# DassHydro-dev/smash

Measured on AMD Instinct MI355X. Metric: cell-timesteps/s, forward+adjoint sweep, higher is better.
Workload: dtype f32

## Files before the change

smash_amd/csrc/smashx.hip:

```cpp
#include "../../include/smashx.h"

#include <hip/hip_runtime.h>
#include <rccl/rccl.h>

#include <dlfcn.h>

#include <algorithm>
#include <functional>
#include <numeric>
#include <cstdio>
#include <cstdlib>
#include <cstring>
#include <string>
#include <vector>

#include "sx_cost.h"
#include "sx_jreg.h"
#include "sx_kernels.h"
#include "sx_ensemble.h"
#include "sx_resident.h"
#include "sx_fields.h"
#include "sx_interception.h"
#include "sx_meanforcing.h"
#include "sx_prcpindices.h"
// ... 199 lines not shown
}

__global__ void k_gauge_rows(float* dst, const float* src, const int* gid, int ng, int nt) {
    const int t = blockIdx.x * blockDim.x + threadIdx.x, g = blockIdx.y;
    if (t < nt && g < ng) dst[(size_t)g * nt + t] = src[(size_t)gid[g] * nt + t];
}


struct RcclApi {
    void* h = nullptr;
    std::string err;
    decltype(&ncclGetUniqueId) GetUniqueId = nullptr;
    decltype(&ncclCommInitRank) CommInitRank = nullptr;
    decltype(&ncclCommDestroy) CommDestroy = nullptr;
    decltype(&ncclSend) Send = nullptr;
    decltype(&ncclRecv) Recv = nullptr;
    decltype(&ncclAllReduce) AllReduce = nullptr;
    decltype(&ncclGroupStart) GroupStart = nullptr;
    decltype(&ncclGroupEnd) GroupEnd = nullptr;
    decltype(&ncclGetErrorString) GetErrorString = nullptr;
    decltype(&ncclCommCount) CommCount = nullptr;
    decltype(&ncclGetVersion) GetVersion = nullptr;
    bool ok() const { return h != nullptr && err.empty(); }
};
RcclApi& rccl() {
    static RcclApi R;
    static bool tried = false;
    if (tried) return R;
    tried = true;
    const char* names[] = {getenv("SMASHX_RCCL_LIB"), "librccl.so.1", "librccl.so", "/opt/rocm/lib/librccl.so.1"};
    for (const char* n : names) {
        if (!n || !n[0]) continue;
        R.h = dlopen(n, RTLD_NOW | RTLD_LOCAL);
        if (R.h) break;
    }
    if (!R.h) { R.err = std::string("librccl.so.1 not found: ") + (dlerror() ? dlerror() : ""); return R; }
#define SX_SYM(f) do { R.f = (decltype(R.f))dlsym(R.h, "nccl" #f); if (!R.f) R.err = "librccl lacks nccl" #f; } while (0)
    SX_SYM(GetUniqueId); SX_SYM(CommInitRank); SX_SYM(CommDestroy); SX_SYM(Send); SX_SYM(Recv); SX_SYM(AllReduce);
    SX_SYM(GroupStart); SX_SYM(GroupEnd); SX_SYM(GetErrorString);
#undef SX_SYM
    R.CommCount = (decltype(R.CommCount))dlsym(R.h, "ncclCommCount");
    R.GetVersion = (decltype(R.GetVersion))dlsym(R.h, "ncclGetVersion");
    return R;
}
#define NCCLCHK(expr)                                                                                   \
    do {                                                                                                \
        ncclResult_t r_ = (expr);                                                                       \
        if (r_ != ncclSuccess)                                                                          \
            return fail(SMASHX_E_HIP, std::string(#expr) + ": " + rccl().GetErrorString(r_) + " (" + __FILE__ + ":" + std::to_string(__LINE__) + ")"); \
    } while (0)

struct SxComm {
    ncclComm_t comm = nullptr;
    int rank = 0, nranks = 1, device = -1;
    hipStream_t stream = nullptr;
    double* d_buf = nullptr;
    std::vector<smashx_plan*> plans;
};
struct PeerSeg { int rank, first, count; };

struct Launch { hipEvent_t a, b; int kind; double cellsteps; };

}

struct smashx_plan {
    smashx_config cfg{};
    SxSchedule sch;
    int n = 0, npad = 0, nt = 0, ng = 0, st = 0;
    long n2 = 0;
    int M = 0;
    int Tc = 0, nchunks = 0;
    bool have_forcing = false, have_options = false, have_qobs = false, uploaded = false;
    bool chunk_ready = false, adj_ready = false;
    smashx_options opt{};
    std::vector<float> wgauge;
    hipStream_t stream = nullptr;
    hipStream_t stream_r = nullptr;
    int Tp = 0;
    bool hi_tape = true;
    int chain_from = 1;
    bool chain_stage = false; SxStageTables stg{}; int stg_blocks = 0, stg_rows_extra = 0; size_t stg_lds = 0;
    float* hrk = nullptr; bool hrk_tried = false, early_adj = true;
    size_t vlds_fwd = 0, vlds_adj = 0;
    std::vector<hipEvent_t> buf_free;
    std::vector<double> round_ncells;
    bool chain_used = false;
    bool chain = true;
    int n_out = 0, n_in = 0;
    int *d_out_x = nullptr, *d_in_x = nullptr;
    float *halo_out = nullptr, *halo_in = nullptr;
    smashx_halo_fn halo_fn = nullptr; void* halo_user = nullptr;
    SxComm* xcomm = nullptr;
    std::vector<PeerSeg> out_segs, in_segs;
    int *d_out_xp = nullptr, *d_in_xp = nullptr;
    float *x_out = nullptr, *x_in = nullptr;
    float* x_keep = nullptr; size_t x_keep_cap = 0;
    std::vector<void*> allocs; std::vector<size_t> alloc_bytes;
    double bytes = 0;
    double hbm_free_at_plan = -1.0, hbm_total = -1.0;
    SxDeviceArrays A{};
    int* d_cell_flat = nullptr;
    int* d_sparse_idx = nullptr;
    float last_jobs_d = 0.f, last_jreg_d = 0.f;
    long n_sparse = 0;
    float* d_stage = nullptr;
    long stage_planes = 0;
    float* d_full[SX_NFIELDS] = {nullptr};
    float* st0[SX_NSSLOTS] = {nullptr};
    float* ckpt = nullptr;
    float* d_prcp = nullptr; float* d_pet = nullptr;
    int* d_ctrl_pos = nullptr; double* d_ctrl = nullptr; size_t ctrl_cap = 0;
    smashx_forcing_layout flay{};
    unsigned short* d_prcp16 = nullptr; float* d_petd = nullptr; float* d_ratio = nullptr; unsigned* d_fstatus = nullptr;
    int ndays = 0; bool petd_open = false;
    std::vector<char> block_seen;
    int ngc = 0;
    std::vector<int> gauge_gid;
    int *d_gauge_gid = nullptr, *d_gauge_flwacc = nullptr;
    float *d_area = nullptr, *d_wgauge = nullptr, *d_qobs = nullptr, *d_qsim_b = nullptr, *d_cost_out = nullptr;
    SxGaugeSums* d_sums = nullptr; SxCostCoef* d_coef = nullptr;
    float* d_med = nullptr; int* d_med_idx = nullptr;
    int med_nslots = 0; int* d_med_slot = nullptr; float* d_medx = nullptr; int* d_medx_idx = nullptr;
    smashx_reduce_fn med_fn = nullptr; void* med_user = nullptr; std::vector<int> med_slot_h;
    float jobs = 0.f;
    struct Signature {
        bool have = false, have_mask = false, ready = false;
        std::vector<float> h_po; std::vector<int> h_mask;
        int maxev_cap = -1;
        int obs_s0 = -1, obs_lds = -1;
        SxSigArgs a{};
        float* d_po = nullptr; int *d_nev = nullptr, *d_ev = nullptr;
        float *d_probe_b = nullptr, *d_probe_gb = nullptr, *d_probe_gd = nullptr, *d_probe_keep = nullptr;
    } sig;
    std::vector<float> h_qobs;
    float* h_qsim_domain = nullptr; float* h_net_prcp_domain = nullptr; int dom_sparse = 0;
    bool dom_q_active = false;
    bool tan_ready = false;
    float* d_qsim_d = nullptr;
    float* d_tanplane[SMASHX_GNP + SMASHX_GNS] = {nullptr};
    bool tiled = false;
    int* d_active = nullptr;
    hipStream_t stream_j = nullptr;
    hipEvent_t ev_j = nullptr;
    float* d_jx[SMASHX_GNP + SMASHX_GNS] = {nullptr};
    float* d_jb[SMASHX_GNP + SMASHX_GNS] = {nullptr};
    float* d_jg[SMASHX_GNP + SMASHX_GNS] = {nullptr};
    float* d_jterm = nullptr; size_t jterm_planes = 0;
    float* d_jsum = nullptr;
    SxJregChains jchains{};
    bool jr_ready = false;
    std::vector<Launch> launches;
    std::vector<hipEvent_t> pool; size_t pool_used = 0;
    hipEvent_t ev0 = nullptr, ev1 = nullptr;
    smashx_timing timing{};
    int last_adjoint = 0;
    std::vector<signed char> h_flwdir;
    std::vector<signed char> h_flwdir_grid;
    struct MeanForcing {
        int state = 0;
        std::string refusal;
        std::vector<int> count;
        std::vector<int> begin;
        std::vector<int> h_list;
        int *d_list = nullptr, *d_begin = nullptr;
        float *d_state = nullptr, *d_mp = nullptr, *d_me = nullptr;
    } mf;
// ... 178 lines not shown
        if ((rc = p->dmalloc(&p->A.xT, (size_t)std::max(p->sch.nxslots, 1) * Tc))) return rc;
        HIPCHK(hipMemsetAsync(p->A.qtT, 0, (size_t)p->npad * Tc * 4, p->stream));
        HIPCHK(hipMemsetAsync(p->A.xT, 0, (size_t)std::max(p->sch.nxslots, 1) * Tc * 4, p->stream));
        p->chunk_ready = true;
    }
    if (p->h_qsim_domain && !p->A.qdT) {
        int rc;
        if ((rc = p->dmalloc(&p->A.qdT, (size_t)p->npad * p->Tc))) return rc;
    }
    if (adjoint && !p->adj_ready) {
        int rc;
        const size_t cs = (size_t)p->npad * p->Tc;
        if (p->A.qsk) { p->dfree(p->A.qsk); p->A.qsk = nullptr; }
        {
            const char* e = getenv("SMASHX_HR_SKEW");
            p->A.hr_skew = e ? atoi(e) != 0 : true;
            if ((rc = p->dmalloc(&p->A.hrT, cs))) return rc;
        }
        if ((rc = p->dmalloc(&p->A.tape_hp, cs))) return rc;
        if ((rc = p->dmalloc(&p->A.tape_hft, cs))) return rc;
        if (st == 5 || ((st == 2 || st == 3) && p->hi_tape)) { if ((rc = p->dmalloc(&p->A.tape_hi, cs))) return rc; }
        else if (st == 2 || st == 3) { if ((rc = p->dmalloc(&p->A.ckpt_hi, cs / SX_HIK))) return rc; }
        if (st == 3) { if ((rc = p->dmalloc(&p->A.tape_hst, cs))) return rc; }
        if (p->nchunks > 1) { if ((rc = p->dmalloc(&p->ckpt, (size_t)p->nchunks * SX_NSSLOTS * p->npad))) return rc; }
        for (int s = 0; s < SX_NSLOTS; ++s) if ((rc = p->dmalloc(&slot_vecs(p, s).grad, (size_t)p->npad))) return rc;
        if ((rc = p->dmalloc(&p->A.qgb, (size_t)std::max(p->ngc, 1) * p->nt))) return rc;
        if ((rc = p->dmalloc(&p->d_qsim_b, (size_t)std::max(p->ng, 1) * p->nt))) return rc;
        p->adj_ready = true;
    }
    if (p->A.ncs > 0 && !p->A.qsk) {
        const size_t need = (size_t)p->A.ncs * 16 * ((size_t)p->Tc / 4 + p->stg_rows_extra + 1);
        size_t fr = 0, tot = 0;
        HIPCHK(hipMemGetInfo(&fr, &tot));
        if ((double)fr > (double)need + 2.0e9) { int rc; if ((rc = p->dmalloc(&p->A.qsk, need / 4))) return rc; }
    }
    if (adjoint && !p->hrk_tried) {
        p->hrk_tried = true;
        const int cf = chain_first(p);
        const char* e = getenv("SMASHX_KEEP_CHAIN_TAPE");
        const bool want = e ? atoi(e) != 0 : true;
        if (const char* ea = getenv("SMASHX_EARLY_ADJ_CHAIN")) p->early_adj = atoi(ea) != 0;
        if (want && p->nchunks > 1 && cf < p->sch.nrounds && !p->tiled && p->n_in == 0 && p->n_out == 0 && p->Tp >= p->Tc) {
            const int kcs0 = p->sch.g_slot_begin[p->sch.round_group_begin[cf]], kncs = p->sch.nslots - kcs0;
            const size_t need = (size_t)(p->nchunks - 1) * (size_t)(p->Tc / 4) * (size_t)kncs * 16;
            size_t fr = 0, tot = 0;
            HIPCHK(hipMemGetInfo(&fr, &tot));
            if (kncs > 0 && (double)fr > (double)need + 2.0e9) {
                int rc; if ((rc = p->dmalloc(&p->hrk, need / 4))) return rc;
                p->A.kcs0 = kcs0; p->A.kncs = kncs;
            }
        }
    }
    return 0;
}

SxDeviceArrays view_at(const smashx_plan* p, int off) {
    SxDeviceArrays B = p->A;
    B.k0 = 0; B.k1 = p->n;
    const size_t q = (size_t)(off / 4);
    B.qtT = p->A.qtT + q * p->npad * 4;
    B.hrk = nullptr;
    if (p->A.hrT) { if (p->A.hr_skew) B.hr_row0 = (int)q; else B.hrT = p->A.hrT + q * p->npad * 4; }
    if (p->A.qdT) B.qdT = p->A.qdT + q * p->npad * 4;
    if (!p->chain) B.qsk = nullptr;
    B.xT = p->A.xT + q * p->A.nx * 4;
    if (p->A.qtdT) B.qtdT = p->A.qtdT + q * p->npad * 4;
    if (p->A.xdT) B.xdT = p->A.xdT + q * p->A.nx * 4;
    if (p->A.tape_hp) B.tape_hp = p->A.tape_hp + (size_t)off * p->npad;
    if (p->A.tape_hft) B.tape_hft = p->A.tape_hft + (size_t)off * p->npad;
    if (p->A.tape_hi) B.tape_hi = p->A.tape_hi + (size_t)off * p->npad;
    if (p->A.ckpt_hi) B.ckpt_hi = p->A.ckpt_hi + (size_t)(off / SX_HIK) * p->npad;
    if (p->A.tape_hst) B.tape_hst = p->A.tape_hst + (size_t)off * p->npad;
    return B;
}

typedef void (*VertKernel)(SxDeviceArrays, int, int);
VertKernel vert_fwd_kernel(int st, bool tape, bool compact) {
#define SX_GR(ST) {sx_k_vert_fwd<ST, false, false>, sx_k_vert_fwd<ST, false, true>, sx_k_vert_fwd<ST, true, false>, sx_k_vert_fwd<ST, true, true>}
    static const VertKernel k[5][4] = {SX_GR(1), SX_GR(2), SX_GR(3), SX_GR(4),
                                       {sx_k_vert_fwd_vic<false, false>, sx_k_vert_fwd_vic<false, true>, sx_k_vert_fwd_vic<true, false>, sx_k_vert_fwd_vic<true, true>}};
#undef SX_GR
    return k[st - 1][2 * tape + compact];
}
VertKernel vert_adj_kernel(int st, bool compact) {
    static const VertKernel k[5][2] = {{sx_k_vert_adj<1, false>, sx_k_vert_adj<1, true>}, {sx_k_vert_adj<2, false>, sx_k_vert_adj<2, true>},
                                       {sx_k_vert_adj<3, false>, sx_k_vert_adj<3, true>}, {sx_k_vert_adj<4, false>, sx_k_vert_adj<4, true>},
                                       {sx_k_vert_adj_vic<false>, sx_k_vert_adj_vic<true>}};
    return k[st - 1][compact];
}
VertKernel vert_tan_kernel(int st) {
    static const VertKernel k[5] = {sx_k_vert_fwd_d<1>, sx_k_vert_fwd_d<2>, sx_k_vert_fwd_d<3>, sx_k_vert_fwd_d<4>, sx_k_vert_fwd_vic_d};
    return k[st - 1];
}
void launch_vert(smashx_plan* p, VertKernel k, int kind, size_t lds, int off, int t0, int T) {
    const SxDeviceArrays B = view_at(p, off);
    if (B.k1 <= B.k0) return;
    const dim3 grid((B.k1 - B.k0 + SX_VBLOCK - 1) / SX_VBLOCK), block(SX_VBLOCK);
    p->mark_begin(kind, p->stream, (double)(B.k1 - B.k0) * T);
    hipLaunchKernelGGL(k, grid, block, lds, p->stream, B, t0, T);
    p->mark_end();
}
void vert_fwd(smashx_plan* p, int off, bool tape, int t0, int T) {
    launch_vert(p, vert_fwd_kernel(p->st, tape, p->A.prcp16 != nullptr), 0, p->st == 5 ? 0 : p->vlds_fwd, off, t0, T);
}
void vert_adj(smashx_plan* p, int off, int t0, int T) {
    launch_vert(p, vert_adj_kernel(p->st, p->A.prcp16 != nullptr), 3, p->st == 5 ? 0 : p->vlds_adj, off, t0, T);
}
void vert_tan(smashx_plan* p, int off, int t0, int T) { launch_vert(p, vert_tan_kernel(p->st), 0, 0, off, t0, T); }
double round_cells(const smashx_plan* p, int r0, int r1) {
    double c = 0.0;
    for (int r = r0; r < r1; ++r) c += p->round_ncells[r];
    return c;
}
int chain_first(const smashx_plan* p) {
    const int nr = p->sch.nrounds;
    return (p->chain && nr - p->chain_from >= 2) ? p->chain_from : nr;
}
void reset_chain_counters(smashx_plan* p, hipStream_t st) {
    (void)hipMemsetAsync(p->A.prog, 0, (size_t)p->sch.ngroups * sizeof(int), st);
    (void)hipMemsetAsync(p->A.prog + p->sch.ngroups + 1, 0, sizeof(int), st);
}
void route_fwd_rounds(smashx_plan* p, int off, bool tape, int t0, int T, hipStream_t st, int r0, int r1, int tan = 0) {
    SxDeviceArrays B = view_at(p, off);
    if (!p->dom_q_active) B.qdT = nullptr;
    if (tan) B.qsk = nullptr;
    const size_t lds = (size_t)2 * p->M * sizeof(float4);
    void (*const k)(SxDeviceArrays, int, int, int, int) = tan == 1 ? sx_k_route_fwd<true, false, 1> : tan == 2 ? sx_k_route_fwd<false, false, 2>
                                                         : tape ? sx_k_route_fwd<true, false> : sx_k_route_fwd<false, false>;
    for (int r = r0; r < r1; ++r) {
        const int g0 = p->sch.round_group_begin[r], ngr = p->sch.round_group_begin[r + 1] - g0;
        p->mark_begin(1, st, round_cells(p, r, r + 1) * T);
        hipLaunchKernelGGL(k, dim3(ngr), dim3(p->M), lds, st, B, g0, g0 + ngr, t0, T);
        p->mark_end();
    }
}
bool route_fwd_chained(smashx_plan* p, int off, bool tape, int t0, int T, hipStream_t st, hipEvent_t inputs_read = nullptr, float* hrk = nullptr) {
    const int nr = p->sch.nrounds, cf = chain_first(p);
    if (cf >= nr) return false;
    SxDeviceArrays B = view_at(p, off);
    if (hrk) { B.hrk = hrk; B.hr_row0 = 0; tape = true; }
    if (!p->dom_q_active) B.qdT = nullptr;
    const size_t lds = (size_t)2 * p->M * sizeof(float4);
    const int g0 = p->sch.round_group_begin[cf], g1 = p->sch.ngroups;
    reset_chain_counters(p, st);
    const int grid = g1 - g0;
    p->mark_begin(5, st, round_cells(p, cf, nr) * T);
    if (B.qsk)
        hipLaunchKernelGGL((sx_k_chain_transpose<true>), dim3((p->stg_blocks + SX_STG_WAVES - 1) / SX_STG_WAVES), dim3(64 * SX_STG_WAVES), p->stg_lds * SX_STG_WAVES, st, B, p->stg, g0, (T + SX_BT - 1) / SX_BT, p->stg_blocks, (int)p->stg_lds);
    const bool early = B.qsk && inputs_read && !B.qdT;
    if (early) (void)hipEventRecord(inputs_read, st);
    if (tape) hipLaunchKernelGGL((sx_k_route_fwd<true, true>), dim3(grid), dim3(p->M), lds, st, B, g0, g1, t0, T);
    else      hipLaunchKernelGGL((sx_k_route_fwd<false, true>), dim3(grid), dim3(p->M), lds, st, B, g0, g1, t0, T);
    p->mark_end();
    p->chain_used = true;
    return early;
}
void route_adj_chained(smashx_plan* p, int off, int t0, int T, hipStream_t st, float* hrk = nullptr, bool launch = true, bool copy = true) {
    const int nr = p->sch.nrounds, cf = chain_first(p);
    if (cf >= nr) return;
    SxDeviceArrays B = view_at(p, off);
    if (hrk) { B.hrk = hrk; B.hr_row0 = 0; }
    const size_t lds = (size_t)2 * p->M * sizeof(float4);
    const int g0 = p->sch.round_group_begin[cf], g1 = p->sch.ngroups;
    const int grid = g1 - g0;
    if (launch) {
        reset_chain_counters(p, st);
        p->mark_begin(6, st, round_cells(p, cf, nr) * T);
        hipLaunchKernelGGL((sx_k_route_adj<true>), dim3(grid), dim3(p->M), lds, st, B, g0, g1, t0, T);
        p->mark_end();
        p->chain_used = true;
    }
    if (copy && B.qsk) {
        p->mark_begin(7, st);
        hipLaunchKernelGGL((sx_k_chain_transpose<false>), dim3((p->stg_blocks + SX_STG_WAVES - 1) / SX_STG_WAVES), dim3(64 * SX_STG_WAVES), p->stg_lds * SX_STG_WAVES, st, B, p->stg, g0, (T + SX_BT - 1) / SX_BT, p->stg_blocks, (int)p->stg_lds);
        p->mark_end();
    }
}
void route_adj_rounds(smashx_plan* p, int off, int t0, int T, hipStream_t st) {
    const SxDeviceArrays B = view_at(p, off);
    const size_t lds = (size_t)2 * p->M * sizeof(float4);
    const int cf = chain_first(p);
    for (int r = cf - 1; r >= 0; --r) {
        const int g0 = p->sch.round_group_begin[r], ngr = p->sch.round_group_begin[r + 1] - g0;
        p->mark_begin(2, st, round_cells(p, r, r + 1) * T);
        hipLaunchKernelGGL((sx_k_route_adj<false>), dim3(ngr), dim3(p->M), lds, st, B, g0, g0 + ngr, t0, T);
        p->mark_end();
    }
}

// ... 80 lines not shown
        sizes[0] = (int)sizeof(smashx_config); sizes[1] = (int)sizeof(smashx_mesh); sizes[2] = (int)sizeof(smashx_options);
        sizes[3] = (int)sizeof(smashx_parameters); sizes[4] = (int)sizeof(smashx_states); sizes[5] = (int)sizeof(smashx_costs);
        sizes[6] = (int)sizeof(smashx_timing);
    }
    return SMASHX_ABI_VERSION;
}

int smashx_device_count(void) {
    int n = 0;
    if (hipGetDeviceCount(&n) != hipSuccess) return 0;
    return n;
}

int smashx_plan_create(const smashx_config* cfg, const smashx_mesh* mesh, smashx_plan** out) {
    if (!cfg || !mesh || !out) return fail(SMASHX_E_ARG, "null argument");
    *out = nullptr;
    if (cfg->structure < 1 || cfg->structure > 5) return fail(SMASHX_E_UNSUPPORTED, "structure must be gr-a/b/c/d or vic-a");
    if (cfg->nrow <= 0 || cfg->ncol <= 0 || cfg->nt <= 0 || cfg->ng < 0 || !(cfg->dt > 0.f) || !(cfg->dx > 0.f))
        return fail(SMASHX_E_ARG, "bad sizes in smashx_config");
    if (!mesh->flwdir || !mesh->flwacc || !mesh->active_cell || (cfg->ng > 0 && (!mesh->gauge_pos || !mesh->area)))
        return fail(SMASHX_E_ARG, "null mesh array");
    int ndev = 0;
    if (hipGetDeviceCount(&ndev) != hipSuccess || ndev <= 0)
        return fail(SMASHX_E_NODEVICE, "no HIP device: libsmashx has no CPU fallback");
    smashx_plan* p = new smashx_plan();
    p->cfg = *cfg;
    if (set_device(p)) { delete p; return SMASHX_E_HIP; }
    p->M = cfg->group_size > 0 ? cfg->group_size : 512;
    if (p->M % 64 != 0 || p->M > SX_MAXGROUP || p->M < 64) { delete p; return fail(SMASHX_E_ARG, "group_size must be a multiple of 64 in [64, 512]"); }
    const bool rect_tile = cfg->tile[1] > cfg->tile[0] && cfg->tile[3] > cfg->tile[2];
    const bool tiled = rect_tile || mesh->owner_mask;
    const int rc0 = sx_build_schedule(cfg->nrow, cfg->ncol, mesh->flwdir, mesh->active_cell, cfg->ng, mesh->gauge_pos, p->M,
                                      rect_tile ? cfg->tile : nullptr, p->sch, mesh->owner_mask, sublevels_env());
    if (rc0 != 0) { std::string e = p->sch.error; delete p; return fail(rc0 == -5 ? SMASHX_E_MESH : SMASHX_E_ARG, e); }
    p->tiled = tiled;
    if (!tiled) {
        p->h_flwdir.resize((size_t)cfg->nrow * cfg->ncol);
        for (size_t c = 0; c < p->h_flwdir.size(); ++c) { const int d = mesh->flwdir[c]; p->h_flwdir[c] = (d >= 1 && d <= 8 && mesh->active_cell[c] == 1) ? (signed char)d : 0; }
        p->h_flwdir_grid.resize(p->h_flwdir.size());
        for (size_t c = 0; c < p->h_flwdir_grid.size(); ++c) { const int d = mesh->flwdir[c]; p->h_flwdir_grid[c] = (d >= 1 && d <= 8) ? (signed char)d : 0; }
    }
    p->n = p->sch.n; p->npad = (p->n + SX_VBLOCK - 1) / SX_VBLOCK * SX_VBLOCK;
    p->nt = cfg->nt; p->ng = cfg->ng; p->st = cfg->structure; p->n2 = (long)cfg->nrow * cfg->ncol;
    int rc = 0;
#define TRY(x) do { rc = (x); if (rc) { smashx_plan_destroy(p); return rc; } } while (0)
    if (hipStreamCreate(&p->stream) != hipSuccess || hipStreamCreate(&p->stream_r) != hipSuccess) { delete p; return fail(SMASHX_E_HIP, "hipStreamCreate failed"); }
    (void)hipEventCreate(&p->ev0); (void)hipEventCreate(&p->ev1);
    if (hipStreamCreate(&p->stream_j) != hipSuccess || hipEventCreate(&p->ev_j) != hipSuccess) { smashx_plan_destroy(p); return fail(SMASHX_E_HIP, "hipStreamCreate failed"); }
    SxDeviceArrays& A = p->A;
    A.n = p->n; A.npad = p->npad; A.nt = p->nt; A.dt = cfg->dt; A.dx = cfg->dx; A.Tc = 0;
    if (getenv("SMASHX_VERBOSE"))
        for (int r = 0; r < p->sch.nrounds; ++r) {
            long slots = 0, inlets = 0, dsum = 0; int dmx = 0;
            const int ga = p->sch.round_group_begin[r], gb = p->sch.round_group_begin[r + 1];
            for (int g = ga; g < gb; ++g) {
                dsum += p->sch.g_dmax[g]; dmx = std::max(dmx, p->sch.g_dmax[g]);
                for (int q = p->sch.g_slot_begin[g]; q < p->sch.g_slot_begin[g + 1]; ++q) { if (p->sch.s_cell[q] == INT_MIN) continue; ++slots; if (p->sch.s_cell[q] < 0) ++inlets; }
            }
            fprintf(stderr, "smashx: routing round %d: %d groups, %ld slots (%ld inlets), depth mean %.1f max %d\n", r, gb - ga, slots, inlets,
                    gb > ga ? (double)dsum / (gb - ga) : 0.0, dmx);
        }
    int *d1, *d2, *d3, *d4, *d5, *d6, *d7, *d8;
    TRY(p->upload_vec(&d1, p->sch.g_slot_begin)); A.g_slot_begin = d1;
    TRY(p->upload_vec(&d2, p->sch.g_dmax)); A.g_dmax = d2;
    TRY(p->upload_vec(&d3, p->sch.s_cell)); A.s_cell = d3;
    TRY(p->upload_vec(&d4, p->sch.s_stage)); A.s_stage = d4;
    TRY(p->upload_vec(&d5, p->sch.s_child)); A.s_child = d5;
    TRY(p->upload_vec(&d6, p->sch.s_ccount)); A.s_ccount = d6;
    { int *e1, *e2; TRY(p->upload_vec(&e1, p->sch.s_sub)); A.s_sub = e1; TRY(p->upload_vec(&e2, p->sch.s_wsub)); A.s_wsub = e2; }
    TRY(p->upload_vec(&d7, p->sch.s_parent)); A.s_parent = d7;
    TRY(p->upload_vec(&d8, p->sch.s_xout)); A.s_xout = d8;
    {
        int *d9, *d10;
        TRY(p->upload_vec(&d9, p->sch.x_prod_group)); A.x_prod = d9;
        TRY(p->upload_vec(&d10, p->sch.x_cons_group)); A.x_cons = d10;
        TRY(p->dmalloc(&A.prog, (size_t)p->sch.ngroups + SX_PROG_EXTRA));
        if (hipMemset(A.prog, 0, ((size_t)p->sch.ngroups + SX_PROG_EXTRA) * sizeof(int)) != hipSuccess) { smashx_plan_destroy(p); return fail(SMASHX_E_HIP, "hipMemset"); }
        A.ngroups = p->sch.ngroups;
        const char* e = getenv("SMASHX_CHAIN_ROUNDS");
        p->chain = !(e && e[0] == '0');
        if (const char* dv = getenv("SMASHX_DEBUG_VLDS")) {
            p->vlds_fwd = p->vlds_adj = (size_t)std::max(0, atoi(dv));
            if (const char* c2 = strchr(dv, ',')) p->vlds_adj = (size_t)std::max(0, atoi(c2 + 1));
        }
        p->round_ncells.assign(p->sch.nrounds, 0.0);
        for (int r = 0; r < p->sch.nrounds; ++r)
            for (int g = p->sch.round_group_begin[r]; g < p->sch.round_group_begin[r + 1]; ++g)
                for (int q = p->sch.g_slot_begin[g]; q < p->sch.g_slot_begin[g + 1]; ++q) p->round_ncells[r] += p->sch.s_cell[q] >= 0;
        const char* cfm = getenv("SMASHX_CHAIN_FROM");
        p->chain_from = cfm ? std::max(0, atoi(cfm)) : 1;
        {
            A.qsk = nullptr; A.cs0 = 0; A.ncs = 0;
            const int cf = chain_first(p);
            {
                int dev = 0, cus = 256;
                if (hipGetDevice(&dev) == hipSuccess) (void)hipDeviceGetAttribute(&cus, hipDeviceAttributeMultiprocessorCount, dev);
                const int nchained = cf < p->sch.nrounds ? p->sch.ngroups - p->sch.round_group_begin[cf] : 0;
                p->chain_stage = nchained >= 2 * cus;
                if (const char* cs = getenv("SMASHX_CHAIN_STAGE")) p->chain_stage = atoi(cs) != 0;
            }
            if (p->chain_stage && cf < p->sch.nrounds) {
                const int gc = p->sch.round_group_begin[cf];
                const int cs0 = p->sch.g_slot_begin[gc], ncs = p->sch.nslots - cs0;
                std::vector<int> slot0, cnt, smn, spr, fg((size_t)std::max(ncs, 1), 0), fs((size_t)std::max(ncs, 1), 0);
                size_t lds = 0;
                int extra = 0;
                for (int g = gc; g < p->sch.ngroups; ++g) {
                    extra = std::max(extra, p->sch.g_dmax[g]);
                    const int sb = p->sch.g_slot_begin[g], m = p->sch.g_slot_begin[g + 1] - sb;
                    for (int o = 0; o < m; o += 64) {
                        const int nl = std::min(64, m - o);
                        int lo = INT_MAX, hi = 0;
                        for (int q = sb + o; q < sb + o + nl; ++q) { lo = std::min(lo, p->sch.s_stage[q]); hi = std::max(hi, p->sch.s_stage[q]); }
                        size_t og = 0, os = 0;
                        for (int q = sb + o; q < sb + o + nl; ++q) {
                            const int d = p->sch.s_stage[q] - lo;
                            fg[q - cs0] = (int)og; og += (size_t)d + 1;
                            fs[q - cs0] = (int)os; os += (size_t)(hi - lo - d) + 1;
                        }
                        lds = std::max(lds, std::max(og, os) * sizeof(float4));
                        slot0.push_back(sb + o); cnt.push_back(nl); smn.push_back(lo); spr.push_back(hi - lo);
                    }
                }
                if (lds * SX_STG_WAVES <= 160 * 1024 && lds <= 64 * 1024 && !slot0.empty()) {
                    int *d0, *d1, *d2, *d3, *d4, *d5;
                    TRY(p->upload_vec(&d0, slot0)); TRY(p->upload_vec(&d1, cnt)); TRY(p->upload_vec(&d2, smn)); TRY(p->upload_vec(&d3, spr));
                    TRY(p->upload_vec(&d4, fg)); TRY(p->upload_vec(&d5, fs));
                    p->stg = SxStageTables{d0, d1, d2, d3, d4, d5};
                    p->stg_blocks = (int)slot0.size(); p->stg_rows_extra = extra; p->stg_lds = (lds + 15) / 16 * 16;
                    static const bool lds_ok = []() {
                        return hipFuncSetAttribute(reinterpret_cast<const void*>(&sx_k_chain_transpose<true>), hipFuncAttributeMaxDynamicSharedMemorySize, 160 * 1024) == hipSuccess
                            && hipFuncSetAttribute(reinterpret_cast<const void*>(&sx_k_chain_transpose<false>), hipFuncAttributeMaxDynamicSharedMemorySize, 160 * 1024) == hipSuccess;
                    }();
                    if (lds_ok || p->stg_lds * SX_STG_WAVES <= 48 * 1024) { A.cs0 = cs0; A.ncs = ncs; }
                    else (void)hipGetLastError();
                }
            }
        }
        A.spin_limit = SX_SPIN_LIMIT; A.mute_group = -1;
        if (const char* sl = getenv("SMASHX_SPIN_LIMIT")) A.spin_limit = std::max(1, atoi(sl));
        if (const char* mg = getenv("SMASHX_DEBUG_MUTE_GROUP")) A.mute_group = atoi(mg);
        if (A.mute_group < -1) A.mute_group = p->sch.round_group_begin[std::min(p->chain_from, p->sch.nrounds - 1)];
        A.gtime = nullptr;
        const char* tr = getenv("SMASHX_TRACE_GROUPS");
        if (tr && tr[0] == '1') {
            TRY(p->dmalloc(&A.gtime, (size_t)4 * p->sch.ngroups));
            if (hipMemset(A.gtime, 0, (size_t)4 * p->sch.ngroups * sizeof(long long)) != hipSuccess) { smashx_plan_destroy(p); return fail(SMASHX_E_HIP, "hipMemset"); }
        }
    }
    TRY(p->upload_vec(&p->d_cell_flat, p->sch.cell_flat));
    TRY(p->upload_vec(&p->d_active, std::vector<int>(mesh->active_cell, mesh->active_cell + p->n2)));
    TRY(p->dmalloc(&p->d_jsum, (size_t)SX_JREG_MAXCHAIN));
    p->n_out = (int)p->sch.out_x.size(); p->n_in = (int)p->sch.in_x.size();
    TRY(p->upload_vec(&p->d_out_x, p->sch.out_x.empty() ? std::vector<int>(1, 0) : p->sch.out_x));
    TRY(p->upload_vec(&p->d_in_x, p->sch.in_x.empty() ? std::vector<int>(1, 0) : p->sch.in_x));
    std::vector<int> facc(p->npad, 1), cg(p->npad, -1);
    for (int k = 0; k < p->n; ++k) facc[k] = mesh->flwacc[p->sch.cell_flat[k]];
    p->gauge_gid.assign(p->ng, -1);
    std::vector<int> gfl(std::max(p->ng, 1), 1);
    for (int g = 0; g < p->ng; ++g) {
        const int k = p->sch.gauge_k[g];
        if (cg[k] < 0) cg[k] = p->ngc++;
        p->gauge_gid[g] = cg[k];
        gfl[g] = mesh->flwacc[p->sch.cell_flat[k]];
    }
    TRY(p->upload_vec(&A.flwacc, facc));
// ... 2587 lines not shown
```

smash_amd/csrc/sx_kernels.h:

```cpp
#pragma once

#include <hip/hip_runtime.h>

#include <climits>

#include "sx_ops.h"
#include "sx_tangent.h"
#include "sx_vic.h"

#define SX_BT 4
#define SX_VBLOCK 256

__device__ __forceinline__ void sx_lds_barrier() {
    __builtin_amdgcn_fence(__ATOMIC_RELEASE, "workgroup", "local");
    __builtin_amdgcn_s_barrier();
    __builtin_amdgcn_fence(__ATOMIC_ACQUIRE, "workgroup", "local");
}

__device__ __forceinline__ void sx_lds_wave_fence() {
    __builtin_amdgcn_fence(__ATOMIC_RELEASE, "workgroup", "local");
    __builtin_amdgcn_wave_barrier();
    __builtin_amdgcn_fence(__ATOMIC_ACQUIRE, "workgroup", "local");
}

// ... 870 lines not shown
            const int w = MU * mw + u;
            const int tbr = w - rstage;
            const bool act = valid && tbr >= 0 && tbr < nb;
            float4* pub = sx_lds + (size_t)(w & 1) * M;
            const float4* prev = sx_lds + (size_t)((w + 1) & 1) * M;
          auto sub_pass = [&](const int sl) {
            if (act && sub == sl) {
                const int tb = nb - 1 - tbr;
                const int tl = tb * SX_BT;
                float4 in4 = cin[u];
                if (par >= 0) in4 = psame ? pub[par] : prev[par];
                if (cell >= 0) {
                    const float hrv[SX_BT] = {chr[u].x, chr[u].y, chr[u].z, chr[u].w};
                    const float inv[SX_BT] = {in4.x, in4.y, in4.z, in4.w};
                    const float sdv[SX_BT] = {csd[u].x, csd[u].y, csd[u].z, csd[u].w};
                    float pb[SX_BT], qtb[SX_BT];
                    float tmpb[SX_BT], qrb[SX_BT], himb[SX_BT], a1b[SX_BT];
                    float nq[SX_BT];
#pragma unroll
                    for (int i = SX_BT - 1; i >= 0; --i) {
                        float q_b = 0.f;
                        if (gid >= 0) q_b = q_b + sdv[i];
                        q_b = q_b + inv[i];
                        nq[i] = (dx * dx) * 0.001f * q_b;
                    }
                    sx_div4(tmpb, nq, ddt);
#pragma unroll
                    for (int i = SX_BT - 1; i >= 0; --i) qrb[i] = f * tmpb[i];
#pragma unroll
                    for (int i = SX_BT - 1; i >= 0; --i) {
                        const bool live = tl + i < T;
                        const float hb1 = hr_b - qrb[i];
                        himb[i] = qrb[i] + a * hb1;
                        a1b[i] = a * hrv[i] * hb1;
                        hr_b = live ? himb[i] : hr_b;
                    }
                    float na[SX_BT], nh[SX_BT], da[SX_BT], dh[SX_BT];
#pragma unroll
                    for (int i = 0; i < SX_BT; ++i) { na[i] = dt * a1b[i]; nh[i] = dt * himb[i]; }
                    sx_div4(da, na, dlr);
                    sx_div4(dh, nh, dden);
#pragma unroll
                    for (int i = SX_BT - 1; i >= 0; --i) {
                        const bool live = tl + i < T;
                        const float lnew = lr_b + da[i];
                        lr_b = live ? lnew : lr_b;
                        pb[i] = (live && hasup) ? dh[i] : 0.f;
                        qtb[i] = live ? tmpb[i] : 0.f;
                    }
                    pub[j] = make_float4(pb[0], pb[1], pb[2], pb[3]);
                    outq[u] = make_float4(qtb[0], qtb[1], qtb[2], qtb[3]);
                } else {
                    outq[u] = in4;
                }
            }
          };
            if (nsubw == 1) sub_pass(0);
            else for (int sl = nsubw - 1; sl >= 0; --sl) { sub_pass(sl); if (sl > 0) sx_lds_wave_fence(); }
            sx_lds_barrier();
            if (CHAIN && u == 0 && j == 0 && mw % PK == 0) { const int done = min(MU * (mw - 1) - dmax, nb); if (done > 0 && g != A.mute_group) sx_publish(A.prog + g, done); }
        }
    }
    if (valid && cell >= 0) { A.hlr_b[cell] = hr_b; A.lr_b[cell] = lr_b; }
    if (A.gtime && j == 0) A.gtime[2 * (A.ngroups + g) + 1] = wall_clock64();
    if (CHAIN) {
        asm volatile("s_waitcnt vmcnt(0)" ::: "memory");
        __builtin_amdgcn_s_barrier();
        if (j == 0 && g != A.mute_group) sx_publish(A.prog + g, nb);
    }
}

template <bool CHAIN>
__global__ __launch_bounds__(SX_MAXGROUP, SX_RLB_A) void sx_k_route_adj(SxDeviceArrays A, int g0, int gend, int t0, int T) {
    if (SX_R_PRIO) __builtin_amdgcn_s_setprio(SX_R_PRIO);
    if (!CHAIN) { sx_route_adj_group<false>(A, g0 + (int)blockIdx.x, g0, gend, t0, T); return; }
    for (;;) {
        const int ticket = sx_next_ticket(A);
        if (ticket >= gend - g0) break;
        sx_route_adj_group<CHAIN>(A, gend - 1 - ticket, g0, gend, t0, T);
    }
}

#ifndef SX_VADJ_WAVES
#define SX_VADJ_WAVES 5
#endif
template <int ST, bool CF>
#ifndef SX_VADJ_WAVES_GRC
#if SX_EXACT_LIBM
#define SX_VADJ_WAVES_GRC 1
#else
#define SX_VADJ_WAVES_GRC 5
#endif
#endif
__global__ __launch_bounds__(SX_VBLOCK, (ST == 2 && CF) ? SX_VADJ_WAVES : (ST == 3 && CF) ? SX_VADJ_WAVES_GRC : 1)
void sx_k_vert_adj(SxDeviceArrays A, int t0, int T) {
    SX_LIBM_INIT();
    const int k = A.k0 + blockIdx.x * SX_VBLOCK + threadIdx.x;
    if (k >= A.k1) return;
    const size_t npad = (size_t)A.npad;
    SxCellParams P;
    P.ci = (ST == 2 || ST == 3) ? A.ci[k] : 1.f;
    P.cp = A.cp[k];
    P.cft = A.cft[k];
    P.cst = (ST == 3) ? A.cst[k] : 1.f;
    P.exc = (ST != 4) ? A.exc[k] : 0.f;
    sx_cell_params_init(P);
    SxAdjParams Q;
    Q.cst_m5 = 1.f;
    sx_pow_m4_m5(P.cft, &P.cft_m4, &Q.cft_m5);
    P.cst_m4 = 1.f;
    if (ST == 3) sx_pow_m4_m5(P.cst, &P.cst_m4, &Q.cst_m5);
    Q.dcft2 = sx_mkdiv(P.cft * P.cft);
    Q.dcst2 = sx_mkdiv(P.cst * P.cst);
    Q.dcp2 = sx_mkdiv(P.cp * P.cp);
    SxCellGrads G;
    G.ci_b = (ST == 2 || ST == 3) ? A.ci_b[k] : 0.f;
    G.cp_b = A.cp_b[k];
    G.cft_b = A.cft_b[k];
    G.cst_b = (ST == 3) ? A.cst_b[k] : 0.f;
    G.exc_b = (ST != 4) ? A.exc_b[k] : 0.f;
    G.hi_b = (ST == 2 || ST == 3) ? A.hi_b[k] : 0.f;
    G.hp_b = A.hp_b[k];
    G.hft_b = A.hft_b[k];
    G.hst_b = (ST == 3) ? A.hst_b[k] : 0.f;
    const unsigned kb = (unsigned)k * 4u;
    SxForcing<CF> F(A, kb, t0 + T - 1);
    float n_hi = 0.f, n_hp = 0.f, n_hft = 0.f, n_hst = 0.f, n_q = 0.f;
    const bool hi_taped = (ST == 2 || ST == 3) && A.tape_hi != nullptr;
    const size_t olast = (size_t)(T > 0 ? T - 1 : 0) * npad;
    const float* r_hi = hi_taped ? A.tape_hi + olast : nullptr;
    const float* r_hp = A.tape_hp + olast;
    const float* r_hft = A.tape_hft + olast;
    const float* r_hst = (ST == 3) ? A.tape_hst + olast : nullptr;
    auto fetch = [&](int tt, bool first) {
        F.template request<SX_VADJ_NT, true>(t0 + tt, first);
        if (hi_taped) { n_hi = sx_row_load<SX_VADJ_NT>(r_hi, kb); r_hi -= npad; }
        n_hp = sx_row_load<SX_VADJ_NT>(r_hp, kb); n_hft = sx_row_load<SX_VADJ_NT>(r_hft, kb);
        r_hp -= npad; r_hft -= npad;
        if (ST == 3) { n_hst = sx_row_load<SX_VADJ_NT>(r_hst, kb); r_hst -= npad; }
        n_q = sx_row_load(A.qtT + (size_t)(tt >> 2) * npad * 4 + (tt & 3), kb * 4u);
    };
    __shared__ float s_hi[(ST == 2 || ST == 3) ? SX_HIK : 1][SX_VBLOCK];
    if (T > 0) fetch(T - 1, true);
    for (int tb = (T - 1) / SX_HIK; tb >= 0; --tb) {
        const int tt0 = tb * SX_HIK, len = min(SX_HIK, T - tt0);
        if ((ST == 2 || ST == 3) && !hi_taped) {
            float fp[SX_HIK], fe[SX_HIK];
#pragma unroll
            for (int j = 0; j < SX_HIK; ++j) sx_forcing_at(A, t0 + tt0 + (j < len ? j : 0), kb, fp[j], fe[j]);
            float h = sx_row_load(A.ckpt_hi + (size_t)tb * npad, kb);
#pragma unroll
            for (int j = 0; j < SX_HIK; ++j) {
                s_hi[j][threadIdx.x] = h;
                if (j < len && fp[j] >= 0.f && fe[j] >= 0.f) { float pn, ei; sx_interception(fp[j], fe[j], P.ci, P.dci, h, pn, ei); }
            }
        }
        for (int tt = tt0 + len - 1; tt >= tt0; --tt) {
            float hit = n_hi, hp = n_hp, hft = n_hft, hst = n_hst, q = n_q;
            F.hold();
            sx_pin1(hp); sx_pin1(hft); sx_pin1(q);
            if (ST == 2 || ST == 3) sx_pin1(hit);
            if (ST == 3) sx_pin1(hst);
            if (tt > 0) fetch(tt - 1, false);
            const float prcp = F.prcp(), pet = F.pet();
            const float hi = (ST == 2 || ST == 3) ? (hi_taped ? hit : s_hi[tt - tt0][threadIdx.x]) : 0.f;
            const bool still = SX_STILL && sx_wave_all(sx_is_still<ST>(prcp, pet, hi, hp));
            sx_vertical_step_b<ST>(P, Q, prcp, pet, hi, hp, hft, hst, q, G, still);
        }
    }
    if (ST == 2 || ST == 3) { A.ci_b[k] = G.ci_b; A.hi_b[k] = G.hi_b; }
    A.cp_b[k] = G.cp_b;
    A.cft_b[k] = G.cft_b;
    if (ST == 3) { A.cst_b[k] = G.cst_b; A.hst_b[k] = G.hst_b; }
    if (ST != 4) A.exc_b[k] = G.exc_b;
    A.hp_b[k] = G.hp_b;
    A.hft_b[k] = G.hft_b;
}
```

Before: 56.73 billion.

## Template vertical adjoint kernel on block size and taped-interception flag

Makes the vertical adjoint kernel a template over its thread-block size (64/128/256, chosen at runtime by an environment variable) and over whether the interception state is taped, so the taped branch is resolved at compile time. It also raises the default occupancy hint for the ST=2 compact-forcing variant from 5 to 6 waves when fast libm is used. The compile-time branch removes dead code and may free registers, and the tighter launch bound may raise occupancy at the cost of register spills. It also multiplies the number of kernel instantiations.

Measured after the change: 57.10 billion (median of 6 runs). Within noise of the previous version (+0.7%).

```diff
diff --git a/smash_amd/csrc/smashx.hip b/smash_amd/csrc/smashx.hip
--- a/smash_amd/csrc/smashx.hip
+++ b/smash_amd/csrc/smashx.hip
@@ -305,6 +305,7 @@
     bool chain_stage = false; SxStageTables stg{}; int stg_blocks = 0, stg_rows_extra = 0; size_t stg_lds = 0;
     float* hrk = nullptr; bool hrk_tried = false, early_adj = true;
     size_t vlds_fwd = 0, vlds_adj = 0;
+    int vadj_block = SX_VADJ_BLOCK;
     std::vector<hipEvent_t> buf_free;
     std::vector<double> round_ncells;
     bool chain_used = false;
@@ -649,20 +650,23 @@
 #undef SX_GR
     return k[st - 1][2 * tape + compact];
 }
-VertKernel vert_adj_kernel(int st, bool compact) {
-    static const VertKernel k[5][2] = {{sx_k_vert_adj<1, false>, sx_k_vert_adj<1, true>}, {sx_k_vert_adj<2, false>, sx_k_vert_adj<2, true>},
-                                       {sx_k_vert_adj<3, false>, sx_k_vert_adj<3, true>}, {sx_k_vert_adj<4, false>, sx_k_vert_adj<4, true>},
-                                       {sx_k_vert_adj_vic<false>, sx_k_vert_adj_vic<true>}};
-    return k[st - 1][compact];
+VertKernel vert_adj_kernel(int st, bool compact, int block, bool hi_taped) {
+#define SX_HI(ST, VB, HIT) {sx_k_vert_adj<ST, false, VB, HIT>, sx_k_vert_adj<ST, true, VB, HIT>}
+#define SX_GR(VB, HIT) {SX_HI(1, VB, true), SX_HI(2, VB, HIT), SX_HI(3, VB, HIT), SX_HI(4, VB, true)}
+    static const VertKernel k[2][3][4][2] = {{SX_GR(256, false), SX_GR(128, false), SX_GR(64, false)}, {SX_GR(256, true), SX_GR(128, true), SX_GR(64, true)}};
+#undef SX_GR
+#undef SX_HI
+    static const VertKernel vic[2] = {sx_k_vert_adj_vic<false>, sx_k_vert_adj_vic<true>};
+    return st == 5 ? vic[compact] : k[hi_taped][block == 256 ? 0 : block == 128 ? 1 : 2][st - 1][compact];
 }
 VertKernel vert_tan_kernel(int st) {
     static const VertKernel k[5] = {sx_k_vert_fwd_d<1>, sx_k_vert_fwd_d<2>, sx_k_vert_fwd_d<3>, sx_k_vert_fwd_d<4>, sx_k_vert_fwd_vic_d};
     return k[st - 1];
 }
-void launch_vert(smashx_plan* p, VertKernel k, int kind, size_t lds, int off, int t0, int T) {
+void launch_vert(smashx_plan* p, VertKernel k, int kind, size_t lds, int off, int t0, int T, int threads = SX_VBLOCK) {
     const SxDeviceArrays B = view_at(p, off);
     if (B.k1 <= B.k0) return;
-    const dim3 grid((B.k1 - B.k0 + SX_VBLOCK - 1) / SX_VBLOCK), block(SX_VBLOCK);
+    const dim3 grid((B.k1 - B.k0 + threads - 1) / threads), block(threads);
     p->mark_begin(kind, p->stream, (double)(B.k1 - B.k0) * T);
     hipLaunchKernelGGL(k, grid, block, lds, p->stream, B, t0, T);
     p->mark_end();
@@ -671,7 +675,8 @@
     launch_vert(p, vert_fwd_kernel(p->st, tape, p->A.prcp16 != nullptr), 0, p->st == 5 ? 0 : p->vlds_fwd, off, t0, T);
 }
 void vert_adj(smashx_plan* p, int off, int t0, int T) {
-    launch_vert(p, vert_adj_kernel(p->st, p->A.prcp16 != nullptr), 3, p->st == 5 ? 0 : p->vlds_adj, off, t0, T);
+    const int threads = p->st == 5 ? SX_VBLOCK : p->vadj_block;
+    launch_vert(p, vert_adj_kernel(p->st, p->A.prcp16 != nullptr, threads, p->A.tape_hi != nullptr), 3, p->st == 5 ? 0 : p->vlds_adj, off, t0, T, threads);
 }
 void vert_tan(smashx_plan* p, int off, int t0, int T) { launch_vert(p, vert_tan_kernel(p->st), 0, 0, off, t0, T); }
 double round_cells(const smashx_plan* p, int r0, int r1) {
@@ -918,6 +923,10 @@
         if (const char* dv = getenv("SMASHX_DEBUG_VLDS")) {
             p->vlds_fwd = p->vlds_adj = (size_t)std::max(0, atoi(dv));
             if (const char* c2 = strchr(dv, ',')) p->vlds_adj = (size_t)std::max(0, atoi(c2 + 1));
+        }
+        if (const char* vb = getenv("SMASHX_VADJ_BLOCK")) {
+            p->vadj_block = atoi(vb);
+            if (p->vadj_block != 64 && p->vadj_block != 128 && p->vadj_block != 256) { smashx_plan_destroy(p); return fail(SMASHX_E_ARG, "SMASHX_VADJ_BLOCK: 64, 128 or 256"); }
         }
         p->round_ncells.assign(p->sch.nrounds, 0.0);
         for (int r = 0; r < p->sch.nrounds; ++r)
diff --git a/smash_amd/csrc/sx_kernels.h b/smash_amd/csrc/sx_kernels.h
--- a/smash_amd/csrc/sx_kernels.h
+++ b/smash_amd/csrc/sx_kernels.h
@@ -976,9 +976,15 @@
 }
 
 #ifndef SX_VADJ_WAVES
+#if SX_EXACT_LIBM
 #define SX_VADJ_WAVES 5
-#endif
-template <int ST, bool CF>
+#else
+#define SX_VADJ_WAVES 6
+#endif
+#endif
+#ifndef SX_VADJ_BLOCK
+#define SX_VADJ_BLOCK 256
+#endif
 #ifndef SX_VADJ_WAVES_GRC
 #if SX_EXACT_LIBM
 #define SX_VADJ_WAVES_GRC 1
@@ -986,10 +992,12 @@
 #define SX_VADJ_WAVES_GRC 5
 #endif
 #endif
-__global__ __launch_bounds__(SX_VBLOCK, (ST == 2 && CF) ? SX_VADJ_WAVES : (ST == 3 && CF) ? SX_VADJ_WAVES_GRC : 1)
+template <int ST, bool CF, int VB = SX_VBLOCK, bool HIT = true>
+__global__ __launch_bounds__(VB, (ST == 2 && CF) ? SX_VADJ_WAVES : (ST == 3 && CF) ? SX_VADJ_WAVES_GRC : 1)
 void sx_k_vert_adj(SxDeviceArrays A, int t0, int T) {
+    static_assert(VB == 64 || VB == 128 || VB == 256, "whole waves, and SX_VBLOCK (the padding of a row) a multiple of the block");
     SX_LIBM_INIT();
-    const int k = A.k0 + blockIdx.x * SX_VBLOCK + threadIdx.x;
+    const int k = A.k0 + blockIdx.x * VB + threadIdx.x;
     if (k >= A.k1) return;
     const size_t npad = (size_t)A.npad;
     SxCellParams P;
@@ -1020,7 +1028,7 @@
     const unsigned kb = (unsigned)k * 4u;
     SxForcing<CF> F(A, kb, t0 + T - 1);
     float n_hi = 0.f, n_hp = 0.f, n_hft = 0.f, n_hst = 0.f, n_q = 0.f;
-    const bool hi_taped = (ST == 2 || ST == 3) && A.tape_hi != nullptr;
+    constexpr bool hi_taped = (ST == 2 || ST == 3) && HIT;
     const size_t olast = (size_t)(T > 0 ? T - 1 : 0) * npad;
     const float* r_hi = hi_taped ? A.tape_hi + olast : nullptr;
     const float* r_hp = A.tape_hp + olast;
@@ -1034,7 +1042,7 @@
         if (ST == 3) { n_hst = sx_row_load<SX_VADJ_NT>(r_hst, kb); r_hst -= npad; }
         n_q = sx_row_load(A.qtT + (size_t)(tt >> 2) * npad * 4 + (tt & 3), kb * 4u);
     };
-    __shared__ float s_hi[(ST == 2 || ST == 3) ? SX_HIK : 1][SX_VBLOCK];
+    __shared__ float s_hi[(ST == 2 || ST == 3) ? SX_HIK : 1][VB];
     if (T > 0) fetch(T - 1, true);
     for (int tb = (T - 1) / SX_HIK; tb >= 0; --tb) {
         const int tt0 = tb * SX_HIK, len = min(SX_HIK, T - tt0);
```
